# sencheng/CoBeL-RL

Hardware: AMD Instinct MI355X
Metric: gridworld env-steps/sec (whole job) (higher is better)
Workload: dtype f32

## Files before the change

cobel-rl_amd/csrc/tabular_pwg.hip:

```cpp
#include <stdlib.h>
#include <string.h>

#include "cobel_common.h"
#include "cobel_policy.h"

namespace {

constexpr int kHashBytes = 128 * 8;
constexpr int kMaxSlices = 8;
constexpr uint32_t kWholeTicket = 0x40000000u;
constexpr uint32_t kWholeThenSlices = 0x80000000u;
constexpr uint32_t kWholeSlice = 0xffu;
constexpr uint32_t kAbortWord = COBEL_TAB_SCRATCH_ABORT_WORD;
constexpr uint32_t kRingSpinLimit = 1u << 22;
struct pwg_args {
  const cobel_wrec* rec;
  const uint16_t* starts;
  const int32_t* start_off;
  int32_t S, n_worlds;
  cobel_tab_run_t r;
  uint64_t thr[16][3];
  float alpha_f, gamma_f, model_lr_f;
  int32_t nl, ng;
  uint32_t* queue;
  uint32_t reserve;
  int32_t n_slices;
  int32_t slice_steps[kMaxSlices];
  uint32_t whole;
  uint32_t* owner;
  uint32_t* tail;
  uint32_t* ring;
  uint32_t ring_stride;
  uint32_t xcc_limit;
};

#if defined(COBEL_PWG_NT)
#define NT_LD(p) __builtin_nontemporal_load(p)
#define NT_ST(v, p) __builtin_nontemporal_store(v, p)
#else
#define NT_LD(p) (*(p))
#define NT_ST(v, p) (*(p) = (v))
#endif

__device__ __forceinline__ void stores_done() { asm volatile("s_waitcnt vmcnt(0)" ::: "memory"); }

#if defined(COBEL_PWG_STAMPS)
__device__ __forceinline__ void pwg_stamp(uint32_t* stamps, uint32_t* prev, int k, int lane) {
  if (lane == 0) {
    const uint32_t now = (uint32_t)__builtin_readcyclecounter();
    atomicAdd(stamps + k, now - *prev);
    *prev = now;
  }
}
#define PWG_STAMP(k) pwg_stamp(stamps, stamp_prev, k, lane)
#else
#define PWG_STAMP(k)
#endif

typedef const __attribute__((address_space(4))) pwg_args* pwg_kargs;
__device__ __forceinline__ pwg_kargs rare_args() {
#if defined(__HIP_DEVICE_COMPILE__)
  pwg_kargs p = (pwg_kargs)__builtin_amdgcn_kernarg_segment_ptr();
  asm volatile("" : "+s"(p));
  return p;
#else
  return nullptr;
#endif
}

template <bool QG, bool POW2>
__device__ __forceinline__ void pwg_instance(const pwg_args& A, const int i, const int step_budget,
                                             unsigned char* const lds, const int lane,
                                             const uint64_t thr_mine, const uint32_t stripe
#if defined(COBEL_PWG_STAMPS)
                                             , uint32_t* stamps, uint32_t* stamp_prev
#endif
                                             ) {
  const int S = A.S;
  float4* const Qs = reinterpret_cast<float4*>(lds);
  float* const Qf = reinterpret_cast<float*>(lds);
  unsigned long long* const H = reinterpret_cast<unsigned long long*>(lds);
  const uint32_t g = A.r.instance_base + (uint32_t)i;
  const int world = (int)(g % (uint32_t)A.n_worlds);
  const uint4* const W4 = reinterpret_cast<const uint4*>(A.rec + (size_t)world * S);
  float4* const Qg = reinterpret_cast<float4*>(A.r.q) + (size_t)i * S;
  float* const Qgf = reinterpret_cast<float*>(Qg);
  uint64_t* const model = A.r.model + (size_t)i * S * 4;
  const uint32_t* const model32 = reinterpret_cast<const uint32_t*>(model);
  const uint32_t SA = (uint32_t)S * 4u;
  uint16_t* const Mg = A.r.model_index + (size_t)i * SA;
  uint32_t succ_sel = (lane & 2) ? 0xffffffffu : 0u, succ_sh = (uint32_t)(lane & 1) * 16u;
  uint32_t SAv = POW2 ? (uint32_t)__builtin_clz(SA) + 1u : SA;
  uint32_t qlane = (uint32_t)(lane & 3);
  asm volatile("" : "+v"(succ_sel), "+v"(succ_sh), "+v"(SAv), "+v"(qlane));
  auto succ_of = [&](uint32_t w0, uint32_t w1) -> uint32_t {
    return (((w1 & succ_sel) | (w0 & ~succ_sel)) >> succ_sh) & 0xffffu;
  };

  int32_t* const inst = A.r.inst + (size_t)i * COBEL_I_WORDS;
  int state = inst[COBEL_I_STATE];
  int step = inst[COBEL_I_STEP];
  int trial = inst[COBEL_I_TRIAL];
  uint32_t ce = (uint32_t)inst[COBEL_I_CTR_ENV];
  uint32_t cp = (uint32_t)inst[COBEL_I_CTR_POLICY];
  uint32_t cm = (uint32_t)inst[COBEL_I_CTR_MEMORY];
  uint32_t iflags = (uint32_t)inst[COBEL_I_FLAGS];
  double trew = *reinterpret_cast<const double*>(inst + COBEL_I_REWARD_LO + (lane & 0));
  asm volatile("" : "+v"(trew));
  uint32_t nonzero = 0u;
  if (QG) {
    for (int s0 = 0; s0 < S; s0 += 512) {
      float4 qv[8];
#pragma unroll
      for (int j = 0; j < 8; ++j) {
        const int s = s0 + j * 64 + lane;
        qv[j] = Qg[s < S ? s : S - 1];
      }
#pragma unroll
      for (int j = 0; j < 8; ++j)
        nonzero |= fbits(qv[j].x) | fbits(qv[j].y) | fbits(qv[j].z) | fbits(qv[j].w);
    }
  } else {
    for (int s0 = 0; s0 < S; s0 += 64) {
      const int s = s0 + lane;
      if (s < S)
        __builtin_amdgcn_global_load_lds(
            (const __attribute__((address_space(1))) void*)(Qg + s),
            (__attribute__((address_space(3))) void*)(Qs + s0), 16, 0, 0);
    }
  }

  const int B = A.r.batch;
#if defined(COBEL_PWG_SSEED)
  auto seed_now = [&]() -> uint64_t {
    uint64_t sd = A.r.seed;
    asm volatile("" : "+s"(sd));
    return sd;
  };
#else
  uint64_t seed_v = A.r.seed;
  asm volatile("" : "+v"(seed_v));
  auto seed_now = [&]() -> uint64_t { return seed_v; };
#endif
  double alpha = A.r.alpha, gamma = A.r.gamma;
  float alpha_f = A.alpha_f, gamma_f = A.gamma_f, mlr_f = A.model_lr_f;
  asm volatile("" : "+v"(alpha), "+v"(gamma), "+v"(alpha_f), "+v"(gamma_f), "+v"(mlr_f));

  uint32_t cw0 = 0, cw1 = 0;
  uint4 cand = {0, 0, 0, 0};
  cobel_u4 blk = {0, 0, 0, 0};
  int refresh_in = 0;
  uint2 mdig = {0u, 0u};
  uint32_t fix_sa = ~0u;
  float fix_r = 0.0f;
  uint32_t idx_cur = 0, mg_cur = 0;

  auto draw_m = [&](uint32_t counter) -> uint32_t {
    const cobel_u4 b = cobel_philox(counter >> 2, (uint32_t)lane, g, COBEL_STREAM_MEMORY, seed_now());
    return cobel_word(b, counter & 3u);
  };
  auto refresh_draws = [&](uint32_t pq) {
    const uint32_t mi = (cm + 1u) >> 2;
    const bool p0 = lane == 62, p1 = lane == 63;
    blk = cobel_philox(p1 ? 2u * pq + 1u : (p0 ? 2u * pq : mi), (p0 || p1) ? 0u : (uint32_t)lane,
                       g, (p0 || p1) ? COBEL_STREAM_POLICY : COBEL_STREAM_MEMORY, seed_now());
  };
  auto enter_state = [&](int s) {
    const uint4 c = W4[s];
    cw0 = rfl(c.x);
    cw1 = rfl(c.y);
    cand = W4[succ_of(cw0, cw1)];
    mdig = *reinterpret_cast<const uint2*>(&Mg[(uint32_t)s * 4u]);
  };
  auto begin_trial = [&]() -> bool {
    const pwg_kargs R = rare_args();
    if (trial >= R->r.trials_target) return false;
    const int start_lo = R->start_off[world];
    const uint32_t start_cnt = (uint32_t)(R->start_off[world + 1] - start_lo);
    state = (int)R->starts[start_lo + (int)cobel_draw_bounded(ce, 0u, g, COBEL_STREAM_ENV, seed_now(),
                                                              start_cnt)];
    ce += 1u;
    step = 0;
    trew = 0.0;
    asm volatile("" : "+v"(trew));
    iflags |= 1u;
    enter_state(state);
    return true;
  };
  auto plan_td = [&](float q, float m, float r, uint32_t nt) -> float {
    const double gnt = gamma * (double)nt;
    double td = (double)r + gnt * (double)m;
    td = td - (double)q;
    return (float)((double)q + alpha * td);
  };
  auto conflict_sets = [&](uint32_t idx, uint32_t ns) -> unsigned long long {
    unsigned long long* const H1 = H;
    unsigned long long* const H2 = H + 64;
    const uint32_t h1 = idx & 63u, h2 = idx >> 6;
    const unsigned long long bit = 1ull << lane;
    atomicOr(&H1[h1], bit);
    atomicOr(&H2[h2], bit);
    __builtin_amdgcn_wave_barrier();
    const ulonglong2* const r4 = reinterpret_cast<const ulonglong2*>(&H1[(ns & 15u) * 4u]);
    const ulonglong2 ra = r4[0], rb = r4[1];
    const unsigned long long cell = H1[h1] & H2[h2];
    const unsigned long long row = ((ra.x | ra.y) | (rb.x | rb.y)) & H2[ns >> 4];
    const unsigned long long cnd = (cell | row) & (bit - 1ull);
    __builtin_amdgcn_wave_barrier();
    H1[h1] = 0ull;
    H2[h2] = 0ull;
    return cnd;
  };
  uint32_t* const Qu = reinterpret_cast<uint32_t*>(lds);
  const uint4* const Qs4u = reinterpret_cast<const uint4*>(lds);
  uint32_t tag_mine = ~(uint32_t)lane;
  auto tag_round = [&](uint32_t idx, uint32_t ns, bool act, bool ch, float q, float qn, int lo) -> int {
    if (ch) atomicMax(&Qu[idx], tag_mine);
    __builtin_amdgcn_wave_barrier();
    uint32_t t = 0u, c2 = 0u;
    if (act) {
      const uint4 r2 = Qs4u[ns];
      c2 = Qu[idx];
      t = max(max(max(r2.x, r2.y), r2.z), max(r2.w, c2));
    }
    const unsigned long long blocked = __builtin_amdgcn_ballot_w64(act && t > tag_mine);
    const int stop = max(blocked ? __ffsll((long long)blocked) - 1 : B, lo + 1);
    if (ch && c2 == tag_mine) Qf[idx] = lane < stop ? qn : q;
    __builtin_amdgcn_wave_barrier();
    return stop;
  };
  auto run_batch_lds = [&](uint32_t idx, uint32_t ns, uint32_t nt, float r) {
    int first;
    {
      const float4 row = Qs[ns];
      const float q = Qf[idx];
      const float qn = plan_td(q, max4(row), r, nt);
      const bool ch = fbits(qn) != fbits(q);
      if (!__builtin_amdgcn_ballot_w64(ch)) return;
      first = tag_round(idx, ns, true, ch, q, qn, 0);
    }
    while (first < B) {
      const bool act = lane >= first;
      float q = 0.0f, qn = 0.0f;
      if (act) {
        const float4 row = Qs[ns];
        q = Qf[idx];
        qn = plan_td(q, max4(row), r, nt);
      }
      const bool ch = act && fbits(qn) != fbits(q);
      if (!__ballot(ch)) return;
      first = tag_round(idx, ns, act, ch, q, qn, first);
    }
  };
  auto run_batch_glb = [&](uint32_t idx, uint32_t ns, uint32_t nt, float r, float4 row, float q) {
    int first = B;
    bool have_conf = false;
    unsigned long long conf = 0ull;
    auto take_writes = [&](unsigned long long pend, float qn) {
      while (__ballot(pend != 0ull)) {
        const int e = pend ? (__ffsll((long long)pend) - 1) : 0;
        const uint32_t ie = (uint32_t)__shfl((int)idx, e);
        const float ve = __shfl(qn, e);
        if (pend) {
          if (ie == idx) q = ve;
          if ((ie >> 2) == ns) {
            const uint32_t c = ie & 3u;
            row.x = c == 0u ? ve : row.x;
            row.y = c == 1u ? ve : row.y;
            row.z = c == 2u ? ve : row.z;
            row.w = c == 3u ? ve : row.w;
          }
          pend &= pend - 1ull;
        }
      }
    };
    {
      const float qn = plan_td(q, max4(row), r, nt);
      const bool ch = fbits(qn) != fbits(q);
      const unsigned long long changed = __builtin_amdgcn_ballot_w64(ch);
      if (!changed) return;
      conf = conflict_sets(idx, ns);
      have_conf = true;
      const unsigned long long blocked = __builtin_amdgcn_ballot_w64((conf & changed) != 0ull);
      if (blocked) first = __ffsll((long long)blocked) - 1;
      if (ch && lane < first) Qgf[idx] = qn;
      if (first < B) {
        const unsigned long long committed = changed & ((1ull << first) - 1ull);
        take_writes(lane >= first ? (conf & committed) : 0ull, qn);
      }
    }
    while (first < B) {
      const bool act = lane >= first;
      float qn = q;
      if (act) qn = plan_td(q, max4(row), r, nt);
      const bool ch = act && fbits(qn) != fbits(q);
      const unsigned long long changed = __ballot(ch);
      int stop = B;
      if (changed) {
        if (!have_conf) {
          conf = conflict_sets(idx, ns);
          have_conf = true;
        }
        const unsigned long long blocked = __ballot(act && (conf & changed) != 0ull);
        if (blocked) stop = __ffsll((long long)blocked) - 1;
        if (ch && lane < stop) Qgf[idx] = qn;
        if (stop < B) {
          const unsigned long long committed = changed & ((1ull << stop) - 1ull);
          take_writes(lane >= stop ? (conf & committed) : 0ull, qn);
        }
      }
      first = stop;
    }
  };

  uint32_t warm;
  {
    const uint32_t off = (uint32_t)lane * 128u, last = SA * 2u - 4u;
    warm = *reinterpret_cast<const uint32_t*>(reinterpret_cast<const char*>(Mg) + (off < last ? off : last));
  }
  bool live = true;
  if (iflags & 1u) enter_state(state);
  else live = begin_trial();
  refresh_draws(cp >> 2);
  {
    const int jp = 3 - (int)(cp & 3u), jm = 4 - (int)((cm + 1u) & 3u);
    refresh_in = jp < jm ? jp : jm;
  }
  idx_cur = lane < B ? cobel_bounded(draw_m(cm), SA) : 0u;
  mg_cur = lane < B ? (uint32_t)Mg[idx_cur] : 0u;
  asm volatile("" ::"v"(warm));
  if (!QG) {
    stores_done();
    for (int s = lane; s < S; s += 64) {
      const float4 qv = Qs[s];
      nonzero |= fbits(qv.x) | fbits(qv.y) | fbits(qv.z) | fbits(qv.w);
    }
  }
  if (QG) {
    for (int b = lane; b < 128; b += 64) H[b] = 0ull;
    __builtin_amdgcn_wave_barrier();
  }
  if (!__ballot(nonzero != 0u)) {
    const uint2* const M2 = reinterpret_cast<const uint2*>(Mg);
    for (int s0 = 0; s0 < S; s0 += 512) {
      uint2 mv[8];
#pragma unroll
      for (int j = 0; j < 8; ++j) {
        const int s = s0 + j * 64 + lane;
        mv[j] = M2[s < S ? s : S - 1];
      }
#pragma unroll
      for (int j = 0; j < 8; ++j) nonzero |= (mv[j].x | mv[j].y) & 0x80008000u;
    }
  }
  if (__ballot(nonzero != 0u)) iflags |= 2u;

  PWG_STAMP(1);
  const int budget0 = step_budget > 0 ? step_budget : 0x7fffffff;
  int budget = budget0;
  uint32_t batches = 0u;
  asm volatile("" : "+v"(batches));

  while (live) {
    if (budget == 0) break;
    budget -= 1;

    const int src_lane = 62 + (int)((cp >> 1) & 1u);
    const uint32_t w0 = rl((cp & 1u) ? blk.z : blk.x, src_lane);
    const uint32_t w1 = rl((cp & 1u) ? blk.w : blk.y, src_lane);
    if (__builtin_expect(refresh_in == 0, 0)) {
      refresh_draws((cp + 1u) >> 2);
      const int jp = 4 - (int)((cp + 1u) & 3u), jm = 4 - (int)((cm + 1u) & 3u);
      refresh_in = jp < jm ? jp : jm;
    }
    refresh_in -= 1;
    cp += 1u;

    const uint32_t succ = succ_of(cw0, cw1);
    float4 srow;
    float qc;
    float4 prow = {0.0f, 0.0f, 0.0f, 0.0f};
    float pq = 0.0f;
    if (QG) {
      stores_done();
      qc = Qgf[(uint32_t)state * 4u + qlane];
      srow = Qg[succ];
      if (lane < B && (iflags & 2u)) {
        prow = Qg[mg_cur & 0x3fffu];
        pq = Qgf[idx_cur];
      }
    } else {
      qc = Qf[(uint32_t)state * 4u + qlane];
      srow = Qs[succ];
    }
    const float smax = max4(srow);

    int a;
    {
      float m;
      asm("s_nop 1\n\t"
          "v_max_f32_dpp %0, %1, %1 quad_perm:[1,0,3,2] row_mask:0xf bank_mask:0xf\n\t"
          "s_nop 1\n\t"
          "v_max_f32_dpp %0, %0, %0 quad_perm:[2,3,0,1] row_mask:0xf bank_mask:0xf"
          : "=&v"(m)
          : "v"(qc));
      const int t = (int)((uint32_t)__ballot(qc == m) & 15u);
      const uint64_t K = cobel_u53(w0, w1);
      const unsigned long long passed = __ballot(thr_mine <= K);
      a = __popcll((passed >> (t * 3)) & 7ull);
    }
    const int ns = (int)next_of(cw0, cw1, a);
    const uint32_t nw0 = rl(cand.x, a), nw1 = rl(cand.y, a);
    const uint32_t r_bits = rl(cand.z, a);
    const float r = __builtin_bit_cast(float, r_bits);
    if (r_bits != 0u) iflags |= 2u;
    const uint32_t end = rl(cand.w, a);
    const float ns_max = __builtin_bit_cast(float, rl(fbits(smax), a));
    const uint32_t nt = 1u - end;
    const uint32_t sa = (uint32_t)state * 4u + (uint32_t)a;
    const bool trial_over = end || (step + 1 >= A.r.steps_per_trial);
    const uint32_t dpair = rfl((a & 2) ? mdig.y : mdig.x);
    const uint32_t dold = (a & 1) ? (dpair >> 16) : (dpair & 0xffffu);
    float R = 0.0f;
    if (__builtin_expect((dold & 0x8000u) != 0u, 0)) {
      R = __builtin_bit_cast(float, rfl(model32[2u * sa]));
    }
    __builtin_amdgcn_sched_barrier(0);
    cand = W4[succ_of(nw0, nw1)];
    const uint2 mdig_next = *reinterpret_cast<const uint2*>(&Mg[(uint32_t)ns * 4u]);

    if (sa == fix_sa) R = fix_r;
    const float d = r - R;
    const float Rn = R + mlr_f * d;
    const uint32_t fresh_idx = sa;
    const float fresh_r = Rn;
    const uint32_t fresh_m = (uint32_t)ns | (nt << 14) | (fbits(Rn) ? 0x8000u : 0u);
    fix_sa = sa;
    fix_r = Rn;
    const float q_sa = __builtin_bit_cast(float, rl(fbits(qc), a));
    const float gnt = nt ? gamma_f : 0.0f;
    float td = r + gnt * ns_max;
    td = td - q_sa;
    const float qn_online = q_sa + alpha_f * td;
    if (lane == 0) {
      if (QG) Qgf[sa] = qn_online;
      else Qf[sa] = qn_online;
      NT_ST(cobel_model_pack(fresh_r, (uint32_t)ns, nt), &model[sa]);
      Mg[sa] = (uint16_t)fresh_m;
    }
    __builtin_amdgcn_wave_barrier();

    trew += (double)r;
    const int s_prev = state;
    state = ns;
    cw0 = nw0;
    cw1 = nw1;

    {
      uint32_t idx_next = 0u, mg_next = 0u;
      const uint32_t m = (idx_cur == fresh_idx) ? fresh_m : mg_cur;
      if (lane < B) {
        float rj = 0.0f;
        idx_next = POW2 ? cobel_word(blk, (cm + 1u) & 3u) >> SAv
                        : cobel_bounded(cobel_word(blk, (cm + 1u) & 3u), SAv);
        mg_next = (uint32_t)Mg[idx_next];
        if (iflags & 2u) {
          batches += 1u;
          if (__builtin_expect((m & 0x8000u) != 0u, 0)) {
            rj = __builtin_bit_cast(float, model32[2u * idx_cur]);
            asm volatile("" : "+v"(rj));
          }
          if (idx_cur == fresh_idx) rj = fresh_r;
          const uint32_t nsj = m & 0x3fffu;
          if (QG) {
            if (__ballot(idx_cur == fresh_idx)) {
              const float4 nrow = {__builtin_bit_cast(float, rl(fbits(srow.x), a)),
                                   __builtin_bit_cast(float, rl(fbits(srow.y), a)),
                                   __builtin_bit_cast(float, rl(fbits(srow.z), a)),
                                   __builtin_bit_cast(float, rl(fbits(srow.w), a))};
              if (idx_cur == fresh_idx) prow = nrow;
            }
            if (idx_cur == sa) pq = qn_online;
            if (nsj == (uint32_t)s_prev) {
              prow.x = a == 0 ? qn_online : prow.x;
              prow.y = a == 1 ? qn_online : prow.y;
              prow.z = a == 2 ? qn_online : prow.z;
              prow.w = a == 3 ? qn_online : prow.w;
            }
            run_batch_glb(idx_cur, nsj, (m >> 14) & 1u, rj, prow, pq);
          } else {
            run_batch_lds(idx_cur, nsj, (m >> 14) & 1u, rj);
          }
        }
        if (idx_next == fresh_idx) mg_next = fresh_m;
      }
      idx_cur = idx_next;
      mg_cur = mg_next;
      mdig = mdig_next;
      cm += 1u;
    }

    if (__builtin_expect(trial_over, 0)) {
      const pwg_kargs R = rare_args();
#define rr (R->r)
      if (lane == 0 && trial >= 0 && trial < rr.trial_cap) {
        const size_t mo = (size_t)stripe * (size_t)rr.trial_cap + (size_t)trial;
        if (rr.lat_sum) atomicAdd(rr.lat_sum + mo, (unsigned long long)step);
        if (rr.lat_cnt) atomicAdd(rr.lat_cnt + mo, 1ull);
        if (rr.reward_sum) atomicAdd(rr.reward_sum + mo, trew);
        if (rr.resp_cnt && trew > 0.0) atomicAdd(rr.resp_cnt + mo, 1ull);
        if (rr.lat_trace) rr.lat_trace[(size_t)i * rr.trial_cap + trial] = step;
      }
#undef rr
      trial += 1;
      iflags &= ~1u;
      if (!begin_trial()) break;
    } else {
      step += 1;
    }
  }

  __builtin_amdgcn_wave_barrier();
  PWG_STAMP(2);
  if (!QG) {
    for (int s0 = 0; s0 < S; s0 += 256) {
      float4 qv[4];
#pragma unroll
      for (int j = 0; j < 4; ++j) {
        const int s = s0 + j * 64 + lane;
        qv[j] = Qs[s < S ? s : S - 1];
      }
#pragma unroll
      for (int j = 0; j < 4; ++j) {
        const int s = s0 + j * 64 + lane;
        if (s < S) Qg[s] = qv[j];
      }
    }
  }
  if (lane == 0) {
    inst[COBEL_I_STATE] = state;
    inst[COBEL_I_STEP] = step;
    inst[COBEL_I_TRIAL] = trial;
    inst[COBEL_I_CTR_ENV] = (int32_t)ce;
    inst[COBEL_I_CTR_POLICY] = (int32_t)cp;
    inst[COBEL_I_CTR_MEMORY] = (int32_t)cm;
    inst[COBEL_I_FLAGS] = (int32_t)(iflags & ~2u);
    const unsigned long long executed = (unsigned long long)(budget0 - budget);
    *reinterpret_cast<double*>(inst + COBEL_I_REWARD_LO) = trew;
    *reinterpret_cast<unsigned long long*>(inst + COBEL_I_STEPS_LO) += executed;
    const pwg_kargs R = rare_args();
    if (R->r.steps_done && executed) atomicAdd(R->r.steps_done, executed);
    if (R->r.batches_done && batches) atomicAdd(R->r.batches_done, (unsigned long long)batches);
  }
  __builtin_amdgcn_wave_barrier();
}

template <bool SLICED, bool POW2>
__global__ __launch_bounds__(1024) void k_tab_pwg(const pwg_args A) {
  extern __shared__ __attribute__((aligned(16))) unsigned char lds_raw[];
  const int lane = (int)(threadIdx.x & 63u);
  const int wave = (int)rfl(threadIdx.x >> 6);
  const int waves = A.nl + A.ng;
  const size_t slice_l = (size_t)A.S * 16;
  const bool qg = wave >= A.nl;
  unsigned char* const lds =
      lds_raw + (qg ? (size_t)A.nl * slice_l + (size_t)(wave - A.nl) * kHashBytes
                    : (size_t)wave * slice_l);
  const uint64_t thr_mine = A.thr[(lane % 48) / 3][lane % 3];
  const uint32_t wave_id = (uint32_t)blockIdx.x * (uint32_t)waves + (uint32_t)wave;
  const uint32_t stripe = A.r.mon_stripes > 1 ? wave_id % (uint32_t)A.r.mon_stripes : 0u;
#if defined(COBEL_PWG_STAMPS)
  uint32_t* const stamps = A.ring + (size_t)8 * A.ring_stride + (size_t)wave_id * 8u;
  uint32_t* const stamp_prev = reinterpret_cast<uint32_t*>(
      lds_raw + (size_t)A.nl * slice_l + (size_t)A.ng * kHashBytes + (size_t)wave * 8);
  if (lane == 0) {
    *stamp_prev = (uint32_t)__builtin_readcyclecounter();
    stamps[7] = (uint32_t)__builtin_amdgcn_s_memrealtime();
  }
#endif
  uint32_t xcc;
  asm volatile("s_getreg_b32 %0, hwreg(HW_REG_XCC_ID)" : "=s"(xcc));
  xcc &= 7u;
  if (SLICED && xcc > A.xcc_limit) return;
  uint32_t tstate = xcc << 8;
  uint32_t t_next = 0xffffffffu;
  for (;;) {
    int i = -1;
    {
      constexpr bool sliced = SLICED;
      uint32_t k0 = tstate & 0xffu;
      const uint32_t x = (tstate >> 8) & 0xffu;
      uint32_t sl = 0u;
      while (k0 < 8u) {
        const uint32_t q = (x + k0) & 7u;
        const uint32_t nq = ((uint32_t)A.r.n + 7u - q) / 8u;
        const uint32_t nw = sliced ? min(nq, A.whole & 0xffffffu) : 0u;
        const uint32_t ns = nq - nw;
        const uint32_t total = SLICED ? ns * (uint32_t)A.n_slices : ns;
        uint32_t t = t_next;
        t_next = 0xffffffffu;
        if (t >= total) t = 0xffffffffu;
        if (t == 0xffffffffu) {
          t = 0x10000000u;
          if (lane == 0 && nq) {
            bool serve = true;
            if (sliced) {
              uint32_t o = __hip_atomic_load(A.owner + q, __ATOMIC_RELAXED, __HIP_MEMORY_SCOPE_AGENT);
              if (o == 0u) {
                o = atomicCAS(A.owner + q, 0u, x + 1u);
                if (o == 0u) o = x + 1u;
              }
              serve = o == x + 1u;
            }
            if (serve) {
              if (qg && nw) {
                const uint32_t b = atomicAdd(A.queue + q * 8u + 1u, 1u);
                if (b < nw) t = kWholeTicket | b;
              }
              if (t == 0x10000000u && !(qg && nw && !(A.whole & kWholeThenSlices)) &&
                  !(qg && __hip_atomic_load(A.queue + q * 8u, __ATOMIC_RELAXED,
                                            __HIP_MEMORY_SCOPE_AGENT) + A.reserve >= total)) {
                t = atomicAdd(A.queue + q * 8u, 1u);
                if (t >= total) {
                  t = 0x10000000u;
                  if (nw) {
                    const uint32_t b = atomicAdd(A.queue + q * 8u + 1u, 1u);
                    if (b < nw) t = kWholeTicket | b;
                  }
                }
              }
            }
          }
          t = rfl(t);
        }
        if (SLICED && (t & kWholeTicket)) {
          i = (int)((t & 0xffffffu) * 8u + q);
          sl = kWholeSlice;
          break;
        }
        if (t < total) {
          if (t < ns) {
            i = (int)((nw + t) * 8u + q);
          } else {
            const uint32_t* const slot = A.ring + (size_t)q * A.ring_stride + (t - ns);
            uint32_t e, spins = 0u;
            while ((e = rfl(__hip_atomic_load(slot, __ATOMIC_RELAXED, __HIP_MEMORY_SCOPE_AGENT))) == 0u) {
              __builtin_amdgcn_s_sleep(32);
              ++spins;
              if (spins >= kRingSpinLimit ||
                  ((spins & 1023u) == 0u &&
                   rfl(__hip_atomic_load(A.queue + kAbortWord, __ATOMIC_RELAXED,
                                         __HIP_MEMORY_SCOPE_AGENT)) != 0u)) {
                if (lane == 0)
                  __hip_atomic_store(A.queue + kAbortWord, 1u, __ATOMIC_RELAXED,
                                     __HIP_MEMORY_SCOPE_AGENT);
                return;
              }
            }
            __builtin_amdgcn_fence(__ATOMIC_ACQUIRE, "agent");
            sl = e >> 24;
            i = (int)(((e & 0xffffffu) - 1u) * 8u + q);
          }
          break;
        }
        k0 += 1u;
      }
      tstate = k0 | (x << 8) | (sl << 16);
    }
#if defined(COBEL_PWG_STAMPS)
    if (i < 0 && lane == 0) {
      stamps[5] = tstate >> 8 & 0xffu;
      stamps[6] = (uint32_t)__builtin_amdgcn_s_memrealtime();
    }
#endif
    if (i < 0) break;
    int budget = A.r.step_budget;
    if (SLICED) {
      const int slice = (int)(tstate >> 16);
#pragma unroll
      for (int j = 0; j < kMaxSlices; ++j)
        if (j == slice) budget = A.slice_steps[j];
    }
#if defined(COBEL_PWG_STAMPS)
    PWG_STAMP(0);
    if (lane == 0) atomicAdd(stamps + 4, 1u);
    if (qg) pwg_instance<true, POW2>(A, i, budget, lds, lane, thr_mine, stripe, stamps, stamp_prev);
    else pwg_instance<false, POW2>(A, i, budget, lds, lane, thr_mine, stripe, stamps, stamp_prev);
    PWG_STAMP(3);
#else
    if (qg) pwg_instance<true, POW2>(A, i, budget, lds, lane, thr_mine, stripe);
    else pwg_instance<false, POW2>(A, i, budget, lds, lane, thr_mine, stripe);
#endif
    if (SLICED) {
      const uint32_t q = (uint32_t)i & 7u;
      const uint32_t sl1 = (tstate >> 16) + 1u;
      const bool more = sl1 < (uint32_t)A.n_slices;
      uint32_t pos = 0u, t = 0xffffffffu;
      if (lane == 0) {
        if (more) pos = atomicAdd(A.tail + q * 8u, 1u);
        if (!qg) t = atomicAdd(A.queue + q * 8u, 1u);
      }
      __builtin_amdgcn_fence(__ATOMIC_RELEASE, "workgroup");
      stores_done();
      if (lane == 0 && more)
        __hip_atomic_store(A.ring + (size_t)q * A.ring_stride + pos,
                           (((uint32_t)i >> 3) + 1u) | (sl1 << 24), __ATOMIC_RELAXED,
                           __HIP_MEMORY_SCOPE_AGENT);
      t_next = rfl(t);
    }
  }
}

}

bool cobel_tab_pwg_plan(const cobel_world* world, const cobel_tab_run_t& r, cobel_tab_plan& plan) {
  static const char* const force = cobel_debug_env("COBEL_DEBUG_PWG");
  const int S = world->n_states;
  if (!plan.midx || plan.lds_pad || (r.flags & (COBEL_F_NO_PWG | COBEL_F_FORCE_WAVE)) ||
      r.occupancy || r.param_index || S * 4 > 4096 || S <= 256 || r.batch > COBEL_MAX_BATCH)
    return false;
  const bool scratch = r.scratch && r.scratch_bytes >= COBEL_TAB_SCRATCH_BYTES(r.n);
  if (!scratch && !world->queue) return false;
  int n_cu = 0;
  size_t total = 0;
  if (cobel_device_limits(world->device, &n_cu, &total) != COBEL_OK) return false;
  const size_t slice_l = (size_t)S * 16;
#if defined(COBEL_PWG_STAMPS)
  total -= 1024;
#endif
  int nl = (int)(total / slice_l);
  if (nl > 16) nl = 16;
  int ng = 0;
  if (force) {
    int a = 0, b = 0;
    if (sscanf(force, "%d,%d", &a, &b) == 2 && a >= 0 && b >= 0 && a + b >= 1 && a + b <= 16 &&
        (size_t)a * slice_l + (size_t)b * kHashBytes <= total) {
      nl = a;
      ng = b;
    }
  } else if (r.flags & COBEL_F_PWG_GLOBAL) {
    nl = 0;
    ng = 16;
  } else if (lds_workgroups_per_cu(slice_l) >= 16) {
    return false;
  }
  plan.kind = COBEL_TAB_KERNEL_PWG;
  plan.lds = (size_t)nl * slice_l + (size_t)ng * kHashBytes;
  plan.wg_per_cu = 1;
  plan.inst_per_wg = nl + ng;
  plan.nl = nl;
  plan.ng = ng;
  return true;
}

static int plan_slices(const cobel_tab_run_t& r, int grid, int n_cu, int nl, int ng, bool scratch,
                       int32_t* steps , uint32_t* whole) {
  const char* const forced = cobel_debug_env("COBEL_DEBUG_PWG_SLICES");
  for (int j = 0; j < kMaxSlices; ++j) steps[j] = 0;
  steps[0] = r.step_budget;
  *whole = 0u;
  if (!scratch || grid < n_cu || r.step_budget < 64) return 1;
  if (forced) {
    int v[kMaxSlices] = {0}, k = 0, sum = 0;
    const char* c = forced;
    while (k < kMaxSlices && *c) {
      v[k] = atoi(c);
      if (v[k] <= 0) break;
      sum += v[k++];
      while (*c && *c != ',') ++c;
      if (*c == ',') ++c;
    }
    if (k >= 1 && sum == r.step_budget) {
      for (int j = 0; j < k; ++j) steps[j] = v[j];
      return k;
    }
    return 1;
  }
  const double rounds = (double)r.n / ((double)grid * (nl + ng));
  const int b = r.step_budget;
  if (rounds < 1.0) return 1;
  if (ng == 0) {
    if (rounds >= 10.0) return 1;
    steps[1] = rounds >= 5.0 ? b / 8 : b / 4;
    steps[0] = b - steps[1];
    return 2;
  }
  if (rounds >= 14.0) return 1;
  if (rounds >= 7.0) {
    steps[1] = b / 8;
    steps[0] = b - steps[1];
    return 2;
  }
  if (rounds >= 3.5) {
    if (rounds >= 4.5 && nl > 0)
      *whole = (uint32_t)(2 * ((ng * grid + 7) / 8)) | kWholeThenSlices;
    steps[1] = b / 4;
    steps[0] = b - steps[1];
    return 2;
  }
  if (rounds >= 1.75 && nl > 0) {
    *whole = (uint32_t)((ng * grid + 7) / 8);
    steps[1] = b / 4;
    steps[0] = b - steps[1];
    return 2;
  }
  steps[2] = b / 8;
  steps[1] = b / 4;
  steps[0] = b - steps[1] - steps[2];
  return 3;
}

int cobel_tab_pwg_launch(const cobel_world* world, const cobel_tab_run_t& r,
                         const cobel_tab_plan& plan, hipStream_t st) {
  const int nl = plan.nl, ng = plan.ng;
  size_t lds = plan.lds;
  pwg_args A;
  A.rec = world->rec;
  A.starts = world->starts;
  A.start_off = world->start_off;
  A.S = world->n_states;
  A.n_worlds = world->n_worlds;
  A.r = r;
  const cobel_eps_consts eps = cobel_make_eps_consts(r.epsilon);
  memcpy(A.thr, eps.thr, sizeof(A.thr));
  A.alpha_f = (float)r.alpha;
  A.gamma_f = (float)r.gamma;
  A.model_lr_f = (float)r.model_lr;
  A.nl = nl;
  A.ng = ng;
  int n_cu = 0;
  size_t lds_cu = 0;
  if (cobel_device_limits(world->device, &n_cu, &lds_cu) != COBEL_OK) return COBEL_E_HIP;
  const int waves = nl + ng;
  int grid = (r.n + waves - 1) / waves;
  if (grid > n_cu) grid = n_cu;
  const bool scratch = r.scratch && r.scratch_bytes >= COBEL_TAB_SCRATCH_BYTES(r.n);
  uint32_t* const base = scratch ? static_cast<uint32_t*>(r.scratch) : world->queue;
  A.queue = base;
  A.owner = scratch ? base + 64 : base;
  A.tail = scratch ? base + 128 : base;
  A.ring = scratch ? base + 256 : base;
  A.n_slices = plan_slices(r, grid, n_cu, nl, ng, scratch, A.slice_steps, &A.whole);
  A.ring_stride = (uint32_t)((r.n + 7) / 8) * (uint32_t)(A.n_slices - 1);
  {
    const char* const w_env = cobel_debug_env("COBEL_DEBUG_PWG_WHOLE");
    if (w_env) A.whole = (uint32_t)strtoul(w_env, nullptr, 0);
    if (nl == 0 || A.n_slices < 2) A.whole = 0u;
  }
  {
    const char* const m_env = cobel_debug_env("COBEL_DEBUG_PWG_XCCLIMIT");
    A.xcc_limit = m_env ? (uint32_t)atoi(m_env) & 7u : 7u;
  }
  {
    static const char* const k_env = cobel_debug_env("COBEL_DEBUG_PWG_RESERVE");
    const double k = k_env ? atof(k_env) : 2.0;
    A.reserve = nl ? (uint32_t)((double)nl * grid * k / 8.0) : 0u;
  }
#if defined(COBEL_PWG_STAMPS)
  lds += 1024;
  COBEL_HIP_TRY(hipMemsetAsync(base, 0, (256 + (size_t)8 * A.ring_stride + (size_t)8 * grid * waves) * 4, st));
#else
  COBEL_HIP_TRY(hipMemsetAsync(base, 0, scratch ? (size_t)kAbortWord * 4 : (size_t)256, st));
  if (A.n_slices > 1)
    COBEL_HIP_TRY(hipMemsetAsync(A.ring, 0, (size_t)8 * A.ring_stride * 4, st));
#endif
  const bool pow2 = (A.S & (A.S - 1)) == 0;
  void (*const kernel)(const pwg_args) =
      A.n_slices > 1 ? (pow2 ? &k_tab_pwg<true, true> : &k_tab_pwg<true, false>)
                     : (pow2 ? &k_tab_pwg<false, true> : &k_tab_pwg<false, false>);
  COBEL_HIP_TRY(cobel_launch(kernel, dim3(grid), dim3(64 * waves), lds, st, A));
  return COBEL_OK;
}
```

Measured before the change: 3.089 billion.

## Unroll env step loop by four with compile-time RNG phase specialization

Wraps the per-step body in a lambda templated on a compile-time phase and, when the policy and memory counters are aligned to four and the Q table is in LDS, runs four steps back to back. Each step selects its Philox words with static indices and refreshes the draw block only at the last phase. This removes the per-step refresh countdown and the dynamic counter arithmetic. It also makes the reward accumulation into trew conditional on a nonzero reward, and reads step through a readfirstlane. The cost is larger code size and register pressure, plus subtle bookkeeping of step, budget and the counters across early trial ends.

```diff
diff --git a/cobel-rl_amd/csrc/tabular_pwg.hip b/cobel-rl_amd/csrc/tabular_pwg.hip
--- a/cobel-rl_amd/csrc/tabular_pwg.hip
+++ b/cobel-rl_amd/csrc/tabular_pwg.hip
@@ -13,6 +13,10 @@
 constexpr uint32_t kWholeSlice = 0xffu;
 constexpr uint32_t kAbortWord = COBEL_TAB_SCRATCH_ABORT_WORD;
 constexpr uint32_t kRingSpinLimit = 1u << 22;
+template <int V>
+struct phase_c {
+  static constexpr int value = V;
+};
 struct pwg_args {
   const cobel_wrec* rec;
   const uint16_t* starts;
@@ -159,11 +163,14 @@
     const cobel_u4 b = cobel_philox(counter >> 2, (uint32_t)lane, g, COBEL_STREAM_MEMORY, seed_now());
     return cobel_word(b, counter & 3u);
   };
-  auto refresh_draws = [&](uint32_t pq) {
-    const uint32_t mi = (cm + 1u) >> 2;
+  auto refresh_draws = [&](uint32_t pq, uint32_t mi) {
     const bool p0 = lane == 62, p1 = lane == 63;
     blk = cobel_philox(p1 ? 2u * pq + 1u : (p0 ? 2u * pq : mi), (p0 || p1) ? 0u : (uint32_t)lane,
                        g, (p0 || p1) ? COBEL_STREAM_POLICY : COBEL_STREAM_MEMORY, seed_now());
+  };
+  auto steps_to_refresh = [&]() -> int {
+    const int jp = 3 - (int)(cp & 3u), jm = 4 - (int)((cm + 1u) & 3u);
+    return jp < jm ? jp : jm;
   };
   auto enter_state = [&](int s) {
     const uint4 c = W4[s];
@@ -321,11 +328,8 @@
   bool live = true;
   if (iflags & 1u) enter_state(state);
   else live = begin_trial();
-  refresh_draws(cp >> 2);
-  {
-    const int jp = 3 - (int)(cp & 3u), jm = 4 - (int)((cm + 1u) & 3u);
-    refresh_in = jp < jm ? jp : jm;
-  }
+  refresh_draws(cp >> 2, (cm + 1u) >> 2);
+  refresh_in = steps_to_refresh();
   idx_cur = lane < B ? cobel_bounded(draw_m(cm), SA) : 0u;
   mg_cur = lane < B ? (uint32_t)Mg[idx_cur] : 0u;
   asm volatile("" ::"v"(warm));
@@ -361,20 +365,25 @@
   uint32_t batches = 0u;
   asm volatile("" : "+v"(batches));
 
-  while (live) {
-    if (budget == 0) break;
-    budget -= 1;
-
-    const int src_lane = 62 + (int)((cp >> 1) & 1u);
-    const uint32_t w0 = rl((cp & 1u) ? blk.z : blk.x, src_lane);
-    const uint32_t w1 = rl((cp & 1u) ? blk.w : blk.y, src_lane);
-    if (__builtin_expect(refresh_in == 0, 0)) {
-      refresh_draws((cp + 1u) >> 2);
-      const int jp = 4 - (int)((cp + 1u) & 3u), jm = 4 - (int)((cm + 1u) & 3u);
-      refresh_in = jp < jm ? jp : jm;
-    }
-    refresh_in -= 1;
-    cp += 1u;
+  auto env_step = [&](auto ph) __attribute__((always_inline)) -> bool {
+    constexpr int PH = decltype(ph)::value;
+    uint32_t w0, w1;
+    if constexpr (PH < 0) {
+      const int src_lane = 62 + (int)((cp >> 1) & 1u);
+      w0 = rl((cp & 1u) ? blk.z : blk.x, src_lane);
+      w1 = rl((cp & 1u) ? blk.w : blk.y, src_lane);
+      if (__builtin_expect(refresh_in == 0, 0)) {
+        refresh_draws((cp + 1u) >> 2, (cm + 1u) >> 2);
+        const int jp = 4 - (int)((cp + 1u) & 3u), jm = 4 - (int)((cm + 1u) & 3u);
+        refresh_in = jp < jm ? jp : jm;
+      }
+      refresh_in -= 1;
+      cp += 1u;
+    } else {
+      w0 = rl((PH & 1) ? blk.z : blk.x, 62 + (PH >> 1));
+      w1 = rl((PH & 1) ? blk.w : blk.y, 62 + (PH >> 1));
+      if constexpr (PH == 3) refresh_draws((cp + 4u) >> 2, (cm + 4u) >> 2);
+    }
 
     const uint32_t succ = succ_of(cw0, cw1);
     float4 srow;
@@ -413,12 +422,16 @@
     const uint32_t nw0 = rl(cand.x, a), nw1 = rl(cand.y, a);
     const uint32_t r_bits = rl(cand.z, a);
     const float r = __builtin_bit_cast(float, r_bits);
-    if (r_bits != 0u) iflags |= 2u;
+    if (__builtin_expect(r_bits != 0u, 0)) {
+      iflags |= 2u;
+      trew += (double)r;
+      asm volatile("" : "+v"(trew));
+    }
     const uint32_t end = rl(cand.w, a);
     const float ns_max = __builtin_bit_cast(float, rl(fbits(smax), a));
     const uint32_t nt = 1u - end;
     const uint32_t sa = (uint32_t)state * 4u + (uint32_t)a;
-    const bool trial_over = end || (step + 1 >= A.r.steps_per_trial);
+    const bool trial_over = end || ((int)rfl((uint32_t)step) + 1 >= A.r.steps_per_trial);
     const uint32_t dpair = rfl((a & 2) ? mdig.y : mdig.x);
     const uint32_t dold = (a & 1) ? (dpair >> 16) : (dpair & 0xffffu);
     float R = 0.0f;
@@ -450,19 +463,19 @@
     }
     __builtin_amdgcn_wave_barrier();
 
-    trew += (double)r;
     const int s_prev = state;
     state = ns;
     cw0 = nw0;
     cw1 = nw1;
 
     {
-      uint32_t idx_next = 0u, mg_next = 0u;
+      uint32_t idx_next = idx_cur, mg_next = mg_cur;
       const uint32_t m = (idx_cur == fresh_idx) ? fresh_m : mg_cur;
       if (lane < B) {
         float rj = 0.0f;
-        idx_next = POW2 ? cobel_word(blk, (cm + 1u) & 3u) >> SAv
-                        : cobel_bounded(cobel_word(blk, (cm + 1u) & 3u), SAv);
+        const uint32_t mword = PH < 0 ? cobel_word(blk, (cm + 1u) & 3u)
+                                      : cobel_word(blk, (uint32_t)(PH + 1) & 3u);
+        idx_next = POW2 ? mword >> SAv : cobel_bounded(mword, SAv);
         mg_next = (uint32_t)Mg[idx_next];
         if (iflags & 2u) {
           batches += 1u;
@@ -497,7 +510,42 @@
       idx_cur = idx_next;
       mg_cur = mg_next;
       mdig = mdig_next;
-      cm += 1u;
+      if constexpr (PH < 0) cm += 1u;
+    }
+    return trial_over;
+  };
+
+  while (live) {
+    bool trial_over;
+    if (!QG && ((cp | cm) & 3u) == 0u && budget >= 4) {
+      uint32_t k = 1u;
+      budget -= 1;
+      trial_over = env_step(phase_c<0>());
+      if (!trial_over) {
+        step += 1;
+        budget -= 1;
+        k = 2u;
+        trial_over = env_step(phase_c<1>());
+        if (!trial_over) {
+          step += 1;
+          budget -= 1;
+          k = 3u;
+          trial_over = env_step(phase_c<2>());
+          if (!trial_over) {
+            step += 1;
+            budget -= 1;
+            k = 4u;
+            trial_over = env_step(phase_c<3>());
+          }
+        }
+      }
+      cp += k;
+      cm += k;
+      refresh_in = steps_to_refresh();
+    } else {
+      if (budget == 0) break;
+      budget -= 1;
+      trial_over = env_step(phase_c<-1>());
     }
 
     if (__builtin_expect(trial_over, 0)) {
```

New measurement: 3.257 billion, median of 6. 1.05x the previous value.
